# marianaGarcez/SpatialFlink

Hardware: AMD Instinct MI355X
Metric: points/sec per window (kNN k=50, range r) at 1/2/4/8 MI355X; % HBM roofline (higher is better)
Workload: dtype f64

## Files before the change

spatialflink_amd/csrc/k_knn.hip:

```cpp
#define GF_TU_NAME k_knn_hip
#include "gf_buildtag.hpp"

#include <type_traits>

#include "gf_geom.hpp"
#include "gf_internal.hpp"

namespace gf {

__device__ __forceinline__ bool classify_cg(const QueryRect& q, double px, double py) {
  const double xs = (px == px) ? px : q.minX;
  const double ys = (py == py) ? py : q.minY;
  const bool inG = q.g_any && in_iv(q.gx, xs) && in_iv(q.gy, ys);
  return inG || (in_iv(q.cgx, xs) && in_iv(q.cgy, ys));
}

template <int METRIC>
__device__ __forceinline__ bool knn_pass(double qx, double qy, const QueryRect& qr, double px, double py,
                                         double sp, double T) {
  const double dx = qx - px, dy = qy - py;
  const double s = dx * dx + dy * dy;
  if (!(s <= sp)) return false;
  if (!classify_cg(qr, px, py)) return false;
  return METRIC == 0 ? true : fdlibm_hypot(dx, dy) <= T;
}
template <int METRIC>
__device__ __forceinline__ double knn_dist(double qx, double qy, double px, double py) {
  const double dx = qx - px, dy = qy - py;
  return METRIC == 0 ? sqrt(dx * dx + dy * dy) : fdlibm_hypot(dx, dy);
}

__device__ __forceinline__ uint64_t okey(int64_t o) { return (uint64_t)o ^ 0x8000000000000000ull; }
__device__ __forceinline__ int64_t from_okey(uint64_t k) { return (int64_t)(k ^ 0x8000000000000000ull); }

struct RecView {
  gf_knn_header* h;
  double* d;
  int64_t* o;
  int64_t* i;
};
__host__ __device__ inline RecView rec_view(void* base, int k) {
  RecView v;
  v.h = (gf_knn_header*)base;
  v.d = (double*)(v.h + 1);
  v.o = (int64_t*)(v.d + k);
  v.i = v.o + k;
  return v;
}

__device__ void sample_finish(KnnState* st, uint32_t* lh, int32_t k, double r, int metric, int64_t bbase) {
  __shared__ uint32_t wsum[kBlock / 64];
  __shared__ int s_last, s_bin;
  __syncthreads();
  for (int j = threadIdx.x; j < kDistBins; j += kBlock)
    if (lh[j]) atomicAdd(&st->hist[j], lh[j]);
  asm volatile("s_waitcnt vmcnt(0)" ::: "memory");
  __syncthreads();
  if (threadIdx.x == 0) {
    const uint32_t t = atomicAdd(&st->ticket, 1u);
    s_last = (t == gridDim.x - 1);
  }
  __syncthreads();
  if (!s_last) return;
  constexpr int kPer = kDistBins / kBlock;
  uint32_t v[kPer];
  uint32_t s = 0;
#pragma unroll
  for (int j = 0; j < kPer; ++j) {
    v[j] = __hip_atomic_load(&st->hist[threadIdx.x * kPer + j], __ATOMIC_RELAXED, __HIP_MEMORY_SCOPE_AGENT);
    s += v[j];
  }
  const int lane = threadIdx.x & 63, wid = threadIdx.x >> 6;
  uint32_t inc = s;
#pragma unroll
  for (int off = 1; off < 64; off <<= 1) {
    const uint32_t t = __shfl_up(inc, off, 64);
    if (lane >= off) inc += t;
  }
  if (lane == 63) wsum[wid] = inc;
  if (threadIdx.x == 0) s_bin = -1;
  __syncthreads();
  uint32_t before = 0;
  for (int w = 0; w < wid; ++w) before += wsum[w];
  const uint32_t excl = before + inc - s;
  const uint32_t kk = (uint32_t)k;
  if (excl < kk && kk <= excl + s) {
    uint32_t run = excl;
    for (int j = 0; j < kPer; ++j) {
      run += v[j];
      if (run >= kk) { s_bin = threadIdx.x * kPer + j; break; }
    }
  }
  __syncthreads();
  if (threadIdx.x == 0) {
    double T = r;
    if (s_bin >= 0) {
      const double up = dist_bin_upper(s_bin, bbase);
      T = up < r ? up : r;
    }
    st->T = T;
    st->s_pre = s_prefilter(T, metric);
    __hip_atomic_store(&st->ticket, 0u, __ATOMIC_RELAXED, __HIP_MEMORY_SCOPE_AGENT);
  }
  for (int j = threadIdx.x; j < kDistBins; j += kBlock) st->hist[j] = 0u;
}

template <int METRIC>
__global__ __launch_bounds__(kBlock) void knn_sample_kernel(KnnSampleArgs a) {
  __shared__ uint32_t lh[kDistBins];
#ifdef GF_TRACE
  if (blockIdx.x == 0 && threadIdx.x == 0) a.st->tr[0] = wall_clock64();
#endif
  if (a.use_hint) {
    const double h = a.st->hint_T;
    if (h > 0.0) {
      if (blockIdx.x == 0 && threadIdx.x == 0) {
        const double T = h < a.r ? h : a.r;
        a.st->T = T;
        a.st->s_pre = s_prefilter(T, a.metric);
      }
      return;
    }
  }
  constexpr int kPairs = kSamplePerBlock / 2 / kBlock;
  for (int j = threadIdx.x; j < kDistBins; j += kBlock) lh[j] = 0u;
  const int64_t npairs = a.n >> 1;
  const int64_t stride = npairs / gridDim.x;
  const int64_t p0 = (int64_t)blockIdx.x * stride;
  const int64_t bbase = dist_bin_base(a.r);
  double2 xv[kPairs], yv[kPairs];
#pragma unroll
  for (int u = 0; u < kPairs; ++u) {
    const int64_t i = 2 * (p0 + u * kBlock + threadIdx.x);
    xv[u] = *reinterpret_cast<const double2*>(a.x + i);
    yv[u] = *reinterpret_cast<const double2*>(a.y + i);
  }
  __syncthreads();
#pragma unroll
  for (int u = 0; u < kPairs; ++u) {
    if (knn_pass<METRIC>(a.qx, a.qy, a.qr, xv[u].x, yv[u].x, a.s_r, a.r))
      atomicAdd(&lh[dist_bin(knn_dist<METRIC>(a.qx, a.qy, xv[u].x, yv[u].x), bbase)], 1u);
    if (knn_pass<METRIC>(a.qx, a.qy, a.qr, xv[u].y, yv[u].y, a.s_r, a.r))
      atomicAdd(&lh[dist_bin(knn_dist<METRIC>(a.qx, a.qy, xv[u].y, yv[u].y), bbase)], 1u);
  }
  sample_finish(a.st, lh, a.k, a.r, a.metric, bbase);
}

hipError_t launch_knn_sample(gf_ctx* ctx, const KnnSampleArgs& a) {
  KTimer t(ctx, GF_K_KNN_SAMPLE);
  if (a.metric == 0)
    hipLaunchKernelGGL(knn_sample_kernel<0>, dim3(kSampleBlocks), dim3(kBlock), 0, ctx->stream, a);
  else
    hipLaunchKernelGGL(knn_sample_kernel<1>, dim3(kSampleBlocks), dim3(kBlock), 0, ctx->stream, a);
  return hipGetLastError();
}

typedef double dbl2 __attribute__((ext_vector_type(2)));

template <int NT>
__device__ __forceinline__ dbl2 ld2(const dbl2* p) {
  if (NT) return __builtin_nontemporal_load(p);
  return *p;
}

template <class C, class Store>
__device__ __forceinline__ void wave_reserve(C* ctr, bool c, Store&& store) {
  const uint64_t m = __ballot(c);
  if (m == 0) return;
  const int lane = threadIdx.x & 63;
  const int leader = __ffsll((unsigned long long)m) - 1;
  C base = 0;
  if (lane == leader) base = atomicAdd(ctr, (C)__popcll(m));
  base = __shfl(base, leader, 64);
  if (c) store(base + (C)__popcll(m & ((1ull << lane) - 1ull)));
}

__device__ __forceinline__ void wave_append(bool c, double d, uint32_t idx, const KnnScanArgs& a) {
  wave_reserve(&a.st->count, c, [&](unsigned long long pos) {
    if (pos < a.cap) {
      a.cand_d[pos] = d;
      a.cand_i[pos] = idx;
      a.cand_o[pos] = a.objID[idx];
    }
  });
}

template <int METRIC, int U>
__device__ __forceinline__ void knn_scan_tile(const KnnScanArgs& a, const dbl2 (&xv)[U], const dbl2 (&yv)[U],
                                              int64_t p0, int64_t wstride, double sp, double T) {
  uint32_t cm = 0;
#pragma unroll
  for (int u = 0; u < U; ++u) {
    cm |= (uint32_t)knn_pass<METRIC>(a.qx, a.qy, a.qr, xv[u].x, yv[u].x, sp, T) << (2 * u);
    cm |= (uint32_t)knn_pass<METRIC>(a.qx, a.qy, a.qr, xv[u].y, yv[u].y, sp, T) << (2 * u + 1);
  }
  if (__ballot(cm != 0)) {
#pragma unroll
    for (int u = 0; u < U; ++u) {
      const uint32_t i0 = (uint32_t)(2 * (p0 + u * wstride));
      const bool c0 = (cm >> (2 * u)) & 1u, c1 = (cm >> (2 * u + 1)) & 1u;
      wave_append(c0, c0 ? knn_dist<METRIC>(a.qx, a.qy, xv[u].x, yv[u].x) : 0.0, i0, a);
      wave_append(c1, c1 ? knn_dist<METRIC>(a.qx, a.qy, xv[u].y, yv[u].y) : 0.0, i0 + 1, a);
    }
  }
}

__device__ __forceinline__ bool x_in_band(double qx, const dbl2& xv, double sp) {
  const double dx0 = qx - xv.x, dx1 = qx - xv.y;
  return (dx0 * dx0 <= sp) | (dx1 * dx1 <= sp);
}

template <int METRIC, int U, int NT>
__device__ __forceinline__ void knn_scan_tile_x(const KnnScanArgs& a, const dbl2 (&xv)[U], const dbl2* py,
                                                int64_t p0, int64_t wstride, double sp, double T) {
  bool bx[U], any = false;
#pragma unroll
  for (int u = 0; u < U; ++u) {
    bx[u] = x_in_band(a.qx, xv[u], sp);
    any |= bx[u];
  }
  if (__ballot(any) == 0) return;
  dbl2 yv[U];
#pragma unroll
  for (int u = 0; u < U; ++u) {
    yv[u].x = NAN; yv[u].y = NAN;
    if (bx[u]) yv[u] = ld2<NT>(py + u * wstride);
  }
  knn_scan_tile<METRIC, U>(a, xv, yv, p0, wstride, sp, T);
}

template <int METRIC, int U, int NT>
__device__ __forceinline__ void knn_scan_body(const KnnScanArgs& a, double sp, double T, int64_t bid, int64_t nblk) {
  const int lane = threadIdx.x & 63;
  const int64_t wstride = nblk * kBlock;
  const int64_t pbeg = a.begin >> 1;
  const int64_t npf = (a.end - a.begin) >> 1;
  const int64_t iters = npf / (U * wstride);
  const int64_t off = bid * kBlock + (threadIdx.x & ~63) + lane;
  const dbl2* px = reinterpret_cast<const dbl2*>(a.x) + pbeg + off;
  const dbl2* py = reinterpret_cast<const dbl2*>(a.y) + pbeg + off;
#ifdef GF_TRACE
  if (threadIdx.x == 0) atomicMin(&a.st->tr[1], (unsigned long long)wall_clock64());
#endif
  dbl2 xv[U];
  if (iters > 0) {
#pragma unroll
    for (int u = 0; u < U; ++u) xv[u] = ld2<NT>(px + u * wstride);
  }
  for (int64_t it = 0; it < iters; ++it) {
    dbl2 xn[U];
    px += U * wstride;
    if (it + 1 < iters) {
#pragma unroll
      for (int u = 0; u < U; ++u) xn[u] = ld2<NT>(px + u * wstride);
    } else {
#pragma unroll
      for (int u = 0; u < U; ++u) { xn[u].x = NAN; xn[u].y = NAN; }
    }
    knn_scan_tile_x<METRIC, U, NT>(a, xv, py, pbeg + off + it * U * wstride, wstride, sp, T);
    py += U * wstride;
#pragma unroll
    for (int u = 0; u < U; ++u) xv[u] = xn[u];
  }
  const int64_t pend = (a.end + 1) >> 1;
  for (int64_t p = pbeg + iters * U * wstride + off; p - lane < pend; p += wstride) {
    const int64_t i = 2 * p;
    dbl2 xt[1], yt[1];
    const bool pair = i + 1 < a.end;
    if (pair) {
      xt[0] = *reinterpret_cast<const dbl2*>(a.x + i);
    } else {
      xt[0].x = i < a.end ? a.x[i] : NAN;
      xt[0].y = NAN;
    }
    yt[0].x = NAN; yt[0].y = NAN;
    const bool bx = x_in_band(a.qx, xt[0], sp);
    if (__ballot(bx) == 0) continue;
    if (bx) {
      if (pair) yt[0] = *reinterpret_cast<const dbl2*>(a.y + i);
      else yt[0].x = a.y[i];
    }
    knn_scan_tile<METRIC, 1>(a, xt, yt, p, wstride, sp, T);
  }
#ifdef GF_TRACE
  __syncthreads();
  if (threadIdx.x == 0) atomicMax(&a.st->tr[2], (unsigned long long)wall_clock64());
#endif
}

template <int METRIC, int U, int NT>
__global__ __launch_bounds__(kBlock) void knn_scan_kernel(KnnScanArgs a) {
  const double sp = a.use_state ? a.st->s_pre : a.s_pre;
  const double T = a.use_state ? a.st->T : a.T;
  knn_scan_body<METRIC, U, NT>(a, sp, T, blockIdx.x, gridDim.x);
}

template <int METRIC>
static void launch_scan_u(gf_ctx* ctx, const KnnScanArgs& a, int blocks, int unroll, int nt) {
  const dim3 g(blocks), b(kBlock);
#define GF_SCAN(U, N) hipLaunchKernelGGL((knn_scan_kernel<METRIC, U, N>), g, b, 0, ctx->stream, a)
  if (nt) {
    if (unroll <= 1) GF_SCAN(1, 1); else if (unroll == 2) GF_SCAN(2, 1); else if (unroll <= 4) GF_SCAN(4, 1); else GF_SCAN(8, 1);
  } else {
    if (unroll <= 1) GF_SCAN(1, 0); else if (unroll == 2) GF_SCAN(2, 0); else if (unroll <= 4) GF_SCAN(4, 0); else GF_SCAN(8, 0);
  }
#undef GF_SCAN
}

hipError_t launch_knn_scan(gf_ctx* ctx, const KnnScanArgs& a, int blocks, int unroll, int nt) {
  KTimer t(ctx, GF_K_KNN_SCAN);
  if (a.metric == 0) launch_scan_u<0>(ctx, a, blocks, unroll, nt);
  else launch_scan_u<1>(ctx, a, blocks, unroll, nt);
  return hipGetLastError();
}

constexpr int kSelT = 256;
static_assert(kSelT == kBlock, "the fused kernel's select block is a scan-sized block");

struct SelFull {
  static constexpr int kCap = 1024, kHBits = 11, kK = kMaxK;
  uint64_t sd[kCap], so[kCap];
  int64_t si[kCap];
  uint64_t rd[kK], ro[kK];
  int64_t ri[kK];
  union {
    uint32_t hist[kDistBins];
    struct {
      uint64_t rund[kSelT], runo[kSelT];
      int64_t runi[kSelT];
      uint64_t hkey[1 << kHBits];
      uint32_t hpos[1 << kHBits];
    };
  };
  uint32_t wsum[kSelT / 64];
  int s_cnt, s_bin, s_maxpos;
  uint32_t s_S, s_below;
  unsigned long long s_rng[4];
};
struct SelLite {
  static constexpr int kCap = 256, kHBits = 9, kK = 256;
  uint64_t sd[kCap], so[kCap];
  int64_t si[kCap];
  uint64_t rd[kK], ro[kK];
  int64_t ri[kK];
  union {
    uint32_t hist[kDistBins];
    struct {
      uint64_t rund[kSelT], runo[kSelT];
      int64_t runi[kSelT];
      uint64_t hkey[1 << kHBits];
      uint32_t hpos[1 << kHBits];
    };
  };
  uint32_t wsum[kSelT / 64];
  int s_cnt, s_bin, s_maxpos;
  uint32_t s_S, s_below;
  unsigned long long s_rng[4];
};
static_assert(SelFull::kCap > kMaxK, "the general path needs room for the running list plus a chunk");
static_assert(sizeof(SelLite) <= 29 * 1024, "fused kernel: 5 blocks per CU must fit the LDS");

__device__ __forceinline__ bool kless(uint64_t ad, uint64_t ao, int64_t ai, uint64_t bd, uint64_t bo, int64_t bi) {
  if (ad != bd) return ad < bd;
  if (ao != bo) return ao < bo;
  return ai < bi;
}

__device__ __forceinline__ void wave_bitonic(uint64_t& d, uint64_t& o, int64_t& i) {
  const int lane = threadIdx.x & 63;
#pragma unroll
  for (int size = 2; size <= 64; size <<= 1) {
#pragma unroll
    for (int stride = size >> 1; stride > 0; stride >>= 1) {
      const uint64_t pd = __shfl_xor(d, stride, 64), po = __shfl_xor(o, stride, 64);
      const int64_t pi = __shfl_xor(i, stride, 64);
      const bool up = (lane & size) == 0;
      const bool lower = (lane & stride) == 0;
      const bool plt = kless(pd, po, pi, d, o, i);
      if ((lower == up) ? plt : !plt) { d = pd; o = po; i = pi; }
    }
  }
}

template <class LDS>
__device__ void sort_regs(LDS& L, uint64_t d, uint64_t o, int64_t i) {
  const int tid = threadIdx.x, lane = tid & 63, w = tid >> 6;
  wave_bitonic(d, o, i);
  L.rund[tid] = d; L.runo[tid] = o; L.runi[tid] = i;
  __syncthreads();
  if (i != INT64_MAX) {
    int rank = lane;
#pragma unroll
    for (int v = 0; v < kSelT / 64; ++v) {
      if (v == w) continue;
      int lo = 0;
#pragma unroll
      for (int step = 32; step > 0; step >>= 1) {
        const int m = 64 * v + lo + step - 1;
        if (kless(L.rund[m], L.runo[m], L.runi[m], d, o, i)) lo += step;
      }
      if (lo == 63 && kless(L.rund[64 * v + 63], L.runo[64 * v + 63], L.runi[64 * v + 63], d, o, i)) lo = 64;
      rank += lo;
    }
    L.sd[rank] = d; L.so[rank] = o; L.si[rank] = i;
  }
  __syncthreads();
}

template <class LDS>
__device__ void bitonic_lds(LDS& L, int P) {
  for (int size = 2; size <= P; size <<= 1) {
    for (int stride = size >> 1; stride > 0; stride >>= 1) {
      for (int t = threadIdx.x; t < (P >> 1); t += kSelT) {
        const int i = 2 * stride * (t / stride) + (t & (stride - 1));
        const int j = i + stride;
        const bool up = (i & size) == 0;
        if (kless(L.sd[j], L.so[j], L.si[j], L.sd[i], L.so[i], L.si[i]) == up) {
          uint64_t td = L.sd[i]; L.sd[i] = L.sd[j]; L.sd[j] = td;
          uint64_t to = L.so[i]; L.so[i] = L.so[j]; L.so[j] = to;
          int64_t ti = L.si[i]; L.si[i] = L.si[j]; L.si[j] = ti;
        }
      }
      __syncthreads();
    }
  }
}

__device__ __forceinline__ int pow2ceil(int v) {
  int p = 2;
  while (p < v) p <<= 1;
  return p;
}

template <class LDS>
__device__ void sort_lds(LDS& L, int cnt) {
  if (cnt <= kSelT) {
    const int tid = threadIdx.x;
    const bool in = tid < cnt;
    const uint64_t d = in ? L.sd[tid] : ~0ull, o = in ? L.so[tid] : ~0ull;
    const int64_t i = in ? L.si[tid] : INT64_MAX;
    __syncthreads();
    sort_regs(L, d, o, i);
  } else {
    const int P = pow2ceil(cnt);
    for (int t = cnt + threadIdx.x; t < P; t += kSelT) { L.sd[t] = ~0ull; L.so[t] = ~0ull; L.si[t] = INT64_MAX; }
    __syncthreads();
    bitonic_lds(L, P);
  }
}

template <class LDS>
__device__ int dedupe_topk(LDS& L, int cnt, int k) {
  constexpr int kH = 1 << LDS::kHBits;
  constexpr int kR = LDS::kCap / kSelT;
  const int tid = threadIdx.x, lane = tid & 63, w = tid >> 6;
  for (int s = tid; s < kH; s += kSelT) { L.hkey[s] = ~0ull; L.hpos[s] = 0xFFFFFFFFu; }
  if (tid == 0) L.s_maxpos = 0x7FFFFFFF;
  __syncthreads();
  uint32_t slot[kR];
#pragma unroll
  for (int r = 0; r < kR; ++r) {
    const int p = r * kSelT + tid;
    slot[r] = 0;
    if (p < cnt) {
      const uint64_t o = L.so[p];
      if (o == ~0ull) {
        atomicMin(&L.s_maxpos, p);
        slot[r] = kH;
      } else {
        uint32_t h = (uint32_t)((o * 0x9E3779B97F4A7C15ull) >> (64 - LDS::kHBits));
        for (;;) {
          const unsigned long long prev = atomicCAS((unsigned long long*)&L.hkey[h], ~0ull, o);
          if (prev == ~0ull || prev == o) break;
          h = (h + 1) & (kH - 1);
        }
        atomicMin(&L.hpos[h], (uint32_t)p);
        slot[r] = h;
      }
    }
  }
  __syncthreads();
  int base = 0;
#pragma unroll
  for (int r = 0; r < kR; ++r) {
    if (r * kSelT < cnt && base < k) {
      const int p = r * kSelT + tid;
      bool keep = false;
      if (p < cnt) keep = (slot[r] == (uint32_t)kH) ? (L.s_maxpos == p) : (L.hpos[slot[r]] == (uint32_t)p);
      const uint64_t m = __ballot(keep);
      if (lane == 0) L.wsum[w] = (uint32_t)__popcll(m);
      __syncthreads();
      int before = base;
      for (int v = 0; v < w; ++v) before += (int)L.wsum[v];
      const int total = (int)(L.wsum[0] + L.wsum[1] + L.wsum[2] + L.wsum[3]);
      const int pos = before + __popcll(m & ((1ull << lane) - 1ull));
      if (keep && pos < k) { L.rd[pos] = L.sd[p]; L.ro[pos] = L.so[p]; L.ri[pos] = L.si[p]; }
      base += total;
      __syncthreads();
    }
  }
  return base < k ? base : k;
}

template <class LDS>
__device__ __forceinline__ void lds_push(LDS& L, bool c, uint64_t d, uint64_t o, int64_t i) {
  wave_reserve(&L.s_cnt, c, [&](int pos) { L.sd[pos] = d; L.so[pos] = o; L.si[pos] = i; });
}

template <class LDS>
__device__ void kth_bin(LDS& L, uint32_t target, uint32_t base) {
  const int tid = threadIdx.x, lane = tid & 63, wid = tid >> 6;
  constexpr int kB = kDistBins / kSelT;
  uint32_t v[kB], s = 0;
#pragma unroll
  for (int j = 0; j < kB; ++j) { v[j] = L.hist[kB * tid + j]; s += v[j]; }
  uint32_t inc = s;
#pragma unroll
  for (int off = 1; off < 64; off <<= 1) {
    const uint32_t t = __shfl_up(inc, off, 64);
    if (lane >= off) inc += t;
  }
  if (lane == 63) L.wsum[wid] = inc;
  __syncthreads();
  const uint32_t total = L.wsum[0] + L.wsum[1] + L.wsum[2] + L.wsum[3];
  uint32_t before = 0;
  for (int w = 0; w < wid; ++w) before += L.wsum[w];
  const uint32_t excl = before + inc - s;
  if (target > total) {
    if (tid == kSelT - 1) { L.s_bin = kDistBins - 1; L.s_S = base + total; L.s_below = base + total - v[kB - 1]; }
  } else if (excl < target && target <= excl + s) {
    uint32_t run = excl;
    for (int j = 0; j < kB; ++j) {
      run += v[j];
      if (run >= target) { L.s_bin = kB * tid + j; L.s_S = base + run; L.s_below = base + run - v[j]; break; }
    }
  }
  __syncthreads();
}

#ifdef GF_TRACE
#define GF_TR(j) do { if (threadIdx.x == 0) tr[j] = wall_clock64(); } while (0)
#else
#define GF_TR(j) do { } while (0)
#endif

template <class LDS, bool GENERAL>
__device__ void knn_select_body(const KnnSelectArgs& a, LDS& L) {
  const int tid = threadIdx.x;
  const int lane = tid & 63;
  const int k = a.k;
  constexpr int kPer = LDS::kCap / kSelT;
#ifdef GF_TRACE
  uint64_t* tr = (uint64_t*)((char*)a.result + sizeof(gf_knn_header) + 24 * (size_t)k);
#endif
  GF_TR(0);
  const unsigned long long count = a.st->count;
  const double T = a.use_state ? a.st->T : a.T;
  double dv[kPer];
  uint32_t iv[kPer];
  int64_t ov[kPer];
#pragma unroll
  for (int j = 0; j < kPer; ++j) {
    const int64_t i = tid + (int64_t)j * kSelT;
    const bool in = (unsigned long long)i < a.cap;
    dv[j] = in ? a.cand_d[i] : 0.0;
    iv[j] = in ? a.cand_i[i] : 0u;
    ov[j] = in ? a.cand_o[i] : 0;
  }
  const bool overflow = count > a.cap;
  const int64_t M = overflow ? 0 : (int64_t)count;
  bool done = overflow;
  int nres = 0;
  GF_TR(1);

  if (!overflow && M <= kSelT) {
    const bool in = tid < M;
    sort_regs(L, in ? dbits(dv[0]) : ~0ull, in ? okey(ov[0]) : ~0ull, in ? (int64_t)iv[0] : INT64_MAX);
    GF_TR(4);
    nres = dedupe_topk(L, (int)M, k);
    done = true;
    GF_TR(5);
  } else if (!overflow) {
    for (int i = tid; i < kDistBins; i += kSelT) L.hist[i] = 0u;
    if (tid == 0) { L.s_cnt = 0; }
    __syncthreads();
    const int64_t bbase = dist_bin_base(T);
    constexpr int kU = GENERAL ? 4 : 2;
    auto each_of = [&](auto&& f, auto with_oi) {
#pragma unroll
      for (int j = 0; j < kPer; ++j) f(tid + (int64_t)j * kSelT < M, dv[j], ov[j], iv[j]);
      for (int64_t i0 = LDS::kCap; i0 < M; i0 += (int64_t)kU * kSelT) {
        double d[kU];
        int64_t o[kU];
        uint32_t x[kU];
#pragma unroll
        for (int u = 0; u < kU; ++u) {
          const int64_t i = i0 + (int64_t)u * kSelT + tid;
          const bool in = i < M;
          d[u] = in ? a.cand_d[i] : 0.0;
          o[u] = in && decltype(with_oi)::value ? a.cand_o[i] : 0;
          x[u] = in && decltype(with_oi)::value ? a.cand_i[i] : 0u;
        }
#pragma unroll
        for (int u = 0; u < kU; ++u) f(i0 + (int64_t)u * kSelT + tid < M, d[u], o[u], x[u]);
      }
    };
    auto each = [&](auto&& f) { each_of(f, std::true_type{}); };
    each_of([&](bool v, double d, int64_t, uint32_t) {
      if (v) atomicAdd(&L.hist[dist_bin(d, bbase)], 1u);
    }, std::false_type{});
    __syncthreads();
    GF_TR(2);
    kth_bin(L, (uint32_t)k, 0u);
    GF_TR(3);
    const int bstar = L.s_bin;
    uint64_t cut_d = ~0ull, cut_o = ~0ull;
    if (L.s_S > (uint32_t)LDS::kCap) {
      uint64_t r0 = ~0ull, r1 = 0ull, r2 = ~0ull, r3 = 0ull;
      each([&](bool v, double d, int64_t o, uint32_t) {
        if (v && dist_bin(d, bbase) == bstar) {
          const uint64_t db = dbits(d), ok = okey(o);
          r0 = db < r0 ? db : r0; r1 = db > r1 ? db : r1;
          r2 = ok < r2 ? ok : r2; r3 = ok > r3 ? ok : r3;
        }
      });
#pragma unroll
      for (int off = 1; off < 64; off <<= 1) {
        const uint64_t t0 = __shfl_xor(r0, off, 64), t1 = __shfl_xor(r1, off, 64);
        const uint64_t t2 = __shfl_xor(r2, off, 64), t3 = __shfl_xor(r3, off, 64);
        r0 = t0 < r0 ? t0 : r0; r1 = t1 > r1 ? t1 : r1; r2 = t2 < r2 ? t2 : r2; r3 = t3 > r3 ? t3 : r3;
      }
      if (tid == 0) { L.s_rng[0] = ~0ull; L.s_rng[1] = 0ull; L.s_rng[2] = ~0ull; L.s_rng[3] = 0ull; }
      for (int i = tid; i < kDistBins; i += kSelT) L.hist[i] = 0u;
      __syncthreads();
      if (lane == 0) {
        atomicMin(&L.s_rng[0], r0); atomicMax(&L.s_rng[1], r1);
        atomicMin(&L.s_rng[2], r2); atomicMax(&L.s_rng[3], r3);
      }
      __syncthreads();
      const bool tie = L.s_rng[0] == L.s_rng[1];
      const uint64_t kmin = tie ? L.s_rng[2] : L.s_rng[0], span = (tie ? L.s_rng[3] : L.s_rng[1]) - kmin;
      const int bits = span ? 64 - __clzll((long long)span) : 0;
      const int shift = bits > 12 ? bits - 12 : 0;
      each([&](bool v, double d, int64_t o, uint32_t) {
        if (v && dist_bin(d, bbase) == bstar) atomicAdd(&L.hist[((tie ? okey(o) : dbits(d)) - kmin) >> shift], 1u);
      });
      __syncthreads();
      const uint32_t below = L.s_below;
      kth_bin(L, (uint32_t)k - below, below);
      const int b2 = L.s_bin;
      const uint64_t cut = b2 >= kDistBins - 1 ? ~0ull : kmin + ((((uint64_t)b2 + 1ull) << shift) - 1ull);
      cut_d = tie ? L.s_rng[0] : cut;
      cut_o = tie ? cut : ~0ull;
    }
    if (L.s_S <= (uint32_t)LDS::kCap) {
      each([&](bool v, double d, int64_t o, uint32_t x) {
        const int b = dist_bin(d, bbase);
        const uint64_t ok = okey(o);
        const bool c = v && (b < bstar || (b == bstar && dbits(d) <= cut_d && ok <= cut_o));
        lds_push(L, c, dbits(d), ok, (int64_t)x);
      });
      __syncthreads();
      GF_TR(4);
      const int cnt = L.s_cnt;
#ifdef GF_TRACE
      if (tid == 0) tr[8] = (uint64_t)cnt;
#endif
      sort_lds(L, cnt);
      nres = dedupe_topk(L, cnt, k);
      done = (nres >= k) || (cnt == M);
      GF_TR(5);
    }
    if (GENERAL && !done) {
      int nr = 0;
      uint64_t md = ~0ull, mo = ~0ull;
      int64_t mi = INT64_MAX;
      for (int64_t i0 = 0; i0 < M; i0 += kSelT) {
        for (int i = tid; i < nr; i += kSelT) { L.sd[i] = L.rd[i]; L.so[i] = L.ro[i]; L.si[i] = L.ri[i]; }
        if (tid == 0) L.s_cnt = nr;
        __syncthreads();
        const int64_t i = i0 + tid;
        bool c = i < M;
        uint64_t d = 0, o = 0;
        int64_t ix = 0;
        if (c) {
          d = dbits(a.cand_d[i]);
          o = okey(a.cand_o[i]);
          ix = (int64_t)a.cand_i[i];
          c = nr < k || kless(d, o, ix, md, mo, mi);
        }
        lds_push(L, c, d, o, ix);
        __syncthreads();
        const int cnt = L.s_cnt;
        if (cnt > nr) {
          sort_lds(L, cnt);
          nr = dedupe_topk(L, cnt, k);
          if (nr == k) { md = L.rd[k - 1]; mo = L.ro[k - 1]; mi = L.ri[k - 1]; }
        }
        __syncthreads();
      }
      nres = nr;
      done = true;
    }
  }
  const bool too_few = done && !overflow && nres < k && T < a.r;
  const int status = (!done || overflow || too_few) ? 1 : 0;
  GF_TR(6);
#ifdef GF_TRACE
  if (tid == 0) {
    tr[9] = a.st->tr[0]; tr[10] = a.st->tr[1]; tr[11] = a.st->tr[2];
    a.st->tr[1] = ~0ull; a.st->tr[2] = 0ull;
  }
#endif
  RecView out = rec_view(a.result, k);
  if (status == 0)
    for (int i = tid; i < nres; i += kSelT) {
      out.d[i] = from_bits(L.rd[i]); out.o[i] = from_okey(L.ro[i]); out.i[i] = L.ri[i] + a.idx_base;
    }
  if (tid == 0) {
    out.h->status = status;
    out.h->n = status ? 0 : nres;
    out.h->k = k;
    out.h->flags = overflow ? 1 : 0;
    out.h->candidates = (int64_t)count;
    out.h->threshold = T;
    a.st->count = 0ull;
    a.st->maybe = 0ull;
    if (a.write_hint) {
      double h;
      if (status == 0) h = nres == k ? fmax(2.0 * from_bits(L.rd[k - 1]), 4.9e-324) : a.r;
      else if (overflow) h = T * sqrt(0.5 * (double)a.cap / (double)count);
      else if (too_few) h = 2.0 * T;
      else h = T;
      a.st->hint_T = h;
    }
  }
}

__global__ __launch_bounds__(kSelT) void knn_select_kernel(KnnSelectArgs a) {
  __shared__ SelFull L;
  knn_select_body<SelFull, true>(a, L);
}

__device__ __forceinline__ int64_t large_count(const KnnLargeArgs& a, int which) {
  const int64_t c = (int64_t)a.cnt[which];
  return c < a.m ? c : a.m;
}

__global__ __launch_bounds__(kBlock) void knn_large_key_kernel(KnnLargeArgs a) {
  const int64_t m = large_count(a, a.pass);
  for (int64_t j = (int64_t)blockIdx.x * kBlock + threadIdx.x; j < m; j += (int64_t)gridDim.x * kBlock) {
    const uint32_t p = a.perm[j];
    uint32_t v;
    switch (a.field) {
      case 0: v = a.ci[p]; break;
      case 1: v = lo32(a.cd[p]); break;
      case 2: v = hi32(a.cd[p]); break;
      case 3: v = (uint32_t)(uint64_t)a.co[p]; break;
      default: v = (uint32_t)((uint64_t)a.co[p] >> 32) ^ 0x80000000u; break;
    }
    a.keys[j] = v;
  }
}

__global__ __launch_bounds__(kBlock) void knn_large_iota_kernel(KnnLargeArgs a) {
  const int64_t m = large_count(a, 0);
  for (int64_t j = (int64_t)blockIdx.x * kBlock + threadIdx.x; j < m; j += (int64_t)gridDim.x * kBlock)
    a.perm[j] = (uint32_t)j;
}

__global__ void knn_large_start_kernel(KnnLargeArgs a) {
  a.cnt[0] = (uint32_t)*a.lane_count;
  a.cnt[1] = 0u;
  *a.lane_count = 0ull;
  *a.lane_maybe = 0ull;
}

__global__ __launch_bounds__(kBlock) void knn_large_first_kernel(KnnLargeArgs a) {
  const int64_t m = large_count(a, 0);
  const int lane = threadIdx.x & 63;
  const int64_t stride = (int64_t)gridDim.x * kBlock;
  for (int64_t j0 = (int64_t)blockIdx.x * kBlock + (threadIdx.x & ~63); j0 < m; j0 += stride) {
    const int64_t j = j0 + lane;
    uint32_t p = 0u;
    bool first = false;
    if (j < m) {
      p = a.perm[j];
      first = j == 0 || a.co[p] != a.co[a.perm[j - 1]];
    }
    wave_reserve(&a.cnt[1], first, [&](uint32_t pos) { a.out[pos] = p; });
  }
}

__global__ __launch_bounds__(kBlock) void knn_large_record_kernel(KnnLargeArgs a) {
  gf_knn_header* h = reinterpret_cast<gf_knn_header*>(a.result);
  const int32_t k = a.k;
  const int32_t n = (int64_t)a.cnt[1] < (int64_t)k ? (int32_t)a.cnt[1] : k;
  double* rd = reinterpret_cast<double*>(h + 1);
  int64_t* ro = reinterpret_cast<int64_t*>(rd + k);
  int64_t* ri = ro + k;
  for (int64_t j = (int64_t)blockIdx.x * kBlock + threadIdx.x; j < n; j += (int64_t)gridDim.x * kBlock) {
    const uint32_t p = a.perm[j];
    rd[j] = a.cd[p];
    ro[j] = a.co[p];
    ri[j] = (int64_t)a.ci[p] + a.idx_base;
  }
  if (blockIdx.x == 0 && threadIdx.x == 0) {
    h->status = 0;
    h->n = n;
    h->k = k;
    h->flags = 0;
    h->candidates = a.cnt[0];
    h->threshold = a.T;
  }
}

static unsigned large_blocks(int64_t items) {
  const int64_t b = (items + kBlock - 1) / kBlock;
  return (unsigned)(b < 1 ? 1 : (b > 2048 ? 2048 : b));
}

hipError_t launch_knn_large(gf_ctx* ctx, int op, const KnnLargeArgs& a) {
  hipStream_t s = ctx->stream;
  const dim3 g(large_blocks(a.m)), b(kBlock);
  switch (op) {
    case 0: hipLaunchKernelGGL(knn_large_iota_kernel, g, b, 0, s, a); break;
    case 1: hipLaunchKernelGGL(knn_large_key_kernel, g, b, 0, s, a); break;
    case 2: hipLaunchKernelGGL(knn_large_first_kernel, g, b, 0, s, a); break;
    case 5: hipLaunchKernelGGL(knn_large_start_kernel, dim3(1), dim3(1), 0, s, a); break;
    default: hipLaunchKernelGGL(knn_large_record_kernel, dim3(large_blocks(a.k)), b, 0, s, a); break;
  }
  return hipGetLastError();
}

hipError_t launch_knn_select(gf_ctx* ctx, const KnnSelectArgs& a) {
  KTimer t(ctx, GF_K_KNN_SELECT);
  hipLaunchKernelGGL(knn_select_kernel, dim3(1), dim3(kSelT), 0, ctx->stream, a);
  return hipGetLastError();
}

struct StridedRecs {
  const char* base;
  size_t stride;
  __device__ const char* operator()(int r) const { return base + (size_t)r * stride; }
};
struct ListRecs {
  const KnnRecList* l;
  __device__ const char* operator()(int r) const { return l->rec[r]; }
};

template <class LDS, class Src>
__device__ void knn_merge_body(int32_t k, const Src& src, int32_t nrec, void* result, LDS& L, int foreign = 0) {
  __shared__ int s_off[kMaxMergeRecs + 1], s_status, s_foreign;
  const int tid = threadIdx.x;
  if (tid == 0) {
    s_foreign = 0;
    int off = 0, st = 0;
    for (int r = 0; r < nrec; ++r) {
      const gf_knn_header* h = (const gf_knn_header*)src(r);
      s_off[r] = off;
      off += h->status == 0 ? h->n : 0;
      st = h->status > st ? h->status : st;
    }
    s_off[nrec] = off;
    s_status = st;
  }
  __syncthreads();
  int nr = 0, r = 0;
  while (r < nrec) {
    for (int i = tid; i < nr; i += kSelT) { L.sd[i] = L.rd[i]; L.so[i] = L.ro[i]; L.si[i] = L.ri[i]; }
    int cnt = nr;
    while (r < nrec && cnt + (s_off[r + 1] - s_off[r]) <= LDS::kCap) {
      RecView in = rec_view((void*)src(r), k);
      const int n = s_off[r + 1] - s_off[r];
      for (int i = tid; i < n; i += kSelT) {
        const int64_t o = in.o[i];
        L.sd[cnt + i] = dbits(in.d[i]); L.so[cnt + i] = okey(o); L.si[cnt + i] = in.i[i];
        if (foreign && o < GF_OBJID_NUMERIC_MIN && o != GF_OBJID_NULL) s_foreign = 1;
      }
      cnt += n;
      ++r;
    }
// ... 649 lines not shown
```

Measured before the change: 796.2 billion.

## Fuse small-candidate sort with hash dedupe and use DPP lane swaps in bitonic

The wave bitonic sort now exchanges lanes with DPP and permlane swaps in place of __shfl_xor, and kless becomes a branchless comparison. For the full layout, the cross-wave merge rank runs its binary searches over the three other waves in lockstep to expose more independent LDS loads. In the general path with at most 256 candidates, a fused sort_dedupe_regs uses an LDS hash table with atomicCAS/atomicMin to keep the first rank per object and bitmask popcounts to compact the top-k, replacing the separate dedupe_topk pass. This aims to cut selection latency and barriers, at the cost of atomic contention, hash probing, and reliance on gfx950 permlane builtins.

Result: no change. 790.7 billion (-0.7%).

```diff
diff --git a/spatialflink_amd/csrc/k_knn.hip b/spatialflink_amd/csrc/k_knn.hip
--- a/spatialflink_amd/csrc/k_knn.hip
+++ b/spatialflink_amd/csrc/k_knn.hip
@@ -319,6 +319,7 @@
 
 struct SelFull {
   static constexpr int kCap = 1024, kHBits = 11, kK = kMaxK;
+  static constexpr bool kLockstep = true;
   uint64_t sd[kCap], so[kCap];
   int64_t si[kCap];
   uint64_t rd[kK], ro[kK];
@@ -339,6 +340,7 @@
 };
 struct SelLite {
   static constexpr int kCap = 256, kHBits = 9, kK = 256;
+  static constexpr bool kLockstep = false;
   uint64_t sd[kCap], so[kCap];
   int64_t si[kCap];
   uint64_t rd[kK], ro[kK];
@@ -361,35 +363,84 @@
 static_assert(sizeof(SelLite) <= 29 * 1024, "fused kernel: 5 blocks per CU must fit the LDS");
 
 __device__ __forceinline__ bool kless(uint64_t ad, uint64_t ao, int64_t ai, uint64_t bd, uint64_t bo, int64_t bi) {
-  if (ad != bd) return ad < bd;
-  if (ao != bo) return ao < bo;
-  return ai < bi;
+  const bool dl = ad < bd, de = ad == bd, ol = ao < bo, oe = ao == bo, il = ai < bi;
+  return dl | (de & (ol | (oe & il)));
+}
+
+template <int CTRL>
+__device__ __forceinline__ uint32_t dpp_mov(uint32_t v) {
+  return (uint32_t)__builtin_amdgcn_mov_dpp((int)v, CTRL, 0xf, 0xf, true);
+}
+template <int STRIDE>
+__device__ __forceinline__ uint32_t lane_xor32(uint32_t v, int lane) {
+  constexpr int kQuadXor1 = 0xB1, kQuadXor2 = 0x4E, kQuadRev = 0x1B, kRowMirror = 0x140, kHalfMirror = 0x141;
+  if constexpr (STRIDE == 1) return dpp_mov<kQuadXor1>(v);
+  else if constexpr (STRIDE == 2) return dpp_mov<kQuadXor2>(v);
+  else if constexpr (STRIDE == 4) return dpp_mov<kQuadRev>(dpp_mov<kHalfMirror>(v));
+  else if constexpr (STRIDE == 8) return dpp_mov<kHalfMirror>(dpp_mov<kRowMirror>(v));
+  else if constexpr (STRIDE == 16) {
+    const auto r = __builtin_amdgcn_permlane16_swap(v, v, false, false);
+    return (lane & 16) ? r[0] : r[1];
+  } else {
+    static_assert(STRIDE == 32, "a wave has 64 lanes");
+    const auto r = __builtin_amdgcn_permlane32_swap(v, v, false, false);
+    return (lane & 32) ? r[0] : r[1];
+  }
+}
+template <int STRIDE>
+__device__ __forceinline__ uint64_t lane_xor(uint64_t v, int lane) {
+  return (uint64_t)lane_xor32<STRIDE>((uint32_t)(v >> 32), lane) << 32 | lane_xor32<STRIDE>((uint32_t)v, lane);
+}
+
+template <int SIZE, int STRIDE>
+__device__ __forceinline__ void bitonic_steps(uint64_t& d, uint64_t& o, int64_t& i, int lane) {
+  const uint64_t pd = lane_xor<STRIDE>(d, lane), po = lane_xor<STRIDE>(o, lane);
+  const int64_t pi = (int64_t)lane_xor<STRIDE>((uint64_t)i, lane);
+  const bool up = (lane & SIZE) == 0;
+  const bool lower = (lane & STRIDE) == 0;
+  const bool plt = kless(pd, po, pi, d, o, i);
+  if ((lower == up) ? plt : !plt) { d = pd; o = po; i = pi; }
+  if constexpr (STRIDE > 1) bitonic_steps<SIZE, STRIDE / 2>(d, o, i, lane);
 }
 
 __device__ __forceinline__ void wave_bitonic(uint64_t& d, uint64_t& o, int64_t& i) {
   const int lane = threadIdx.x & 63;
-#pragma unroll
-  for (int size = 2; size <= 64; size <<= 1) {
-#pragma unroll
-    for (int stride = size >> 1; stride > 0; stride >>= 1) {
-      const uint64_t pd = __shfl_xor(d, stride, 64), po = __shfl_xor(o, stride, 64);
-      const int64_t pi = __shfl_xor(i, stride, 64);
-      const bool up = (lane & size) == 0;
-      const bool lower = (lane & stride) == 0;
-      const bool plt = kless(pd, po, pi, d, o, i);
-      if ((lower == up) ? plt : !plt) { d = pd; o = po; i = pi; }
-    }
-  }
+  bitonic_steps<2, 1>(d, o, i, lane);
+  bitonic_steps<4, 2>(d, o, i, lane);
+  bitonic_steps<8, 4>(d, o, i, lane);
+  bitonic_steps<16, 8>(d, o, i, lane);
+  bitonic_steps<32, 16>(d, o, i, lane);
+  bitonic_steps<64, 32>(d, o, i, lane);
 }
 
 template <class LDS>
-__device__ void sort_regs(LDS& L, uint64_t d, uint64_t o, int64_t i) {
-  const int tid = threadIdx.x, lane = tid & 63, w = tid >> 6;
-  wave_bitonic(d, o, i);
-  L.rund[tid] = d; L.runo[tid] = o; L.runi[tid] = i;
-  __syncthreads();
-  if (i != INT64_MAX) {
-    int rank = lane;
+__device__ __forceinline__ int merged_rank(const LDS& L, uint64_t d, uint64_t o, int64_t i, int lane, int w) {
+  int rank = lane;
+  if constexpr (LDS::kLockstep) {
+    constexpr int kF = kSelT / 64 - 1;
+    int base[kF], lo[kF];
+    bool all[kF];
+#pragma unroll
+    for (int u = 0; u < kF; ++u) {
+      base[u] = 64 * ((w + 1 + u) & (kSelT / 64 - 1));
+      lo[u] = 0;
+      const int m = base[u] + 63;
+      all[u] = kless(L.rund[m], L.runo[m], L.runi[m], d, o, i);
+    }
+#pragma unroll
+    for (int step = 32; step > 0; step >>= 1) {
+      bool below[kF];
+#pragma unroll
+      for (int u = 0; u < kF; ++u) {
+        const int m = base[u] + lo[u] + step - 1;
+        below[u] = kless(L.rund[m], L.runo[m], L.runi[m], d, o, i);
+      }
+#pragma unroll
+      for (int u = 0; u < kF; ++u) lo[u] += below[u] ? step : 0;
+    }
+#pragma unroll
+    for (int u = 0; u < kF; ++u) rank += all[u] ? 64 : lo[u];
+  } else {
 #pragma unroll
     for (int v = 0; v < kSelT / 64; ++v) {
       if (v == w) continue;
@@ -402,9 +453,68 @@
       if (lo == 63 && kless(L.rund[64 * v + 63], L.runo[64 * v + 63], L.runi[64 * v + 63], d, o, i)) lo = 64;
       rank += lo;
     }
+  }
+  return rank;
+}
+
+template <class LDS>
+__device__ void sort_regs(LDS& L, uint64_t d, uint64_t o, int64_t i) {
+  const int tid = threadIdx.x, lane = tid & 63, w = tid >> 6;
+  wave_bitonic(d, o, i);
+  L.rund[tid] = d; L.runo[tid] = o; L.runi[tid] = i;
+  __syncthreads();
+  if (i != INT64_MAX) {
+    const int rank = merged_rank(L, d, o, i, lane, w);
     L.sd[rank] = d; L.so[rank] = o; L.si[rank] = i;
   }
   __syncthreads();
+}
+
+template <class LDS>
+__device__ int sort_dedupe_regs(LDS& L, uint64_t d, uint64_t o, int64_t i, int k) {
+  constexpr int kHB = 9, kH = 1 << kHB;
+  static_assert(kHB <= LDS::kHBits && kH >= 2 * kSelT, "load factor <= 1/2 inside the layout's table");
+  const int tid = threadIdx.x, lane = tid & 63, w = tid >> 6;
+  for (int s = tid; s < kH; s += kSelT) { L.hkey[s] = ~0ull; L.hpos[s] = 0xFFFFFFFFu; }
+  if (tid < 4) L.s_rng[tid] = 0ull;
+  if (tid == 0) L.s_maxpos = 0x7FFFFFFF;
+  wave_bitonic(d, o, i);
+  L.rund[tid] = d; L.runo[tid] = o; L.runi[tid] = i;
+  __syncthreads();
+  int rank = -1;
+  uint32_t slot = 0;
+  if (i != INT64_MAX) {
+    rank = merged_rank(L, d, o, i, lane, w);
+    if (o == ~0ull) {
+      atomicMin(&L.s_maxpos, rank);
+      slot = kH;
+    } else {
+      uint32_t h = (uint32_t)((o * 0x9E3779B97F4A7C15ull) >> (64 - kHB));
+      for (;;) {
+        const unsigned long long prev = atomicCAS((unsigned long long*)&L.hkey[h], ~0ull, o);
+        if (prev == ~0ull || prev == o) break;
+        h = (h + 1) & (kH - 1);
+      }
+      atomicMin(&L.hpos[h], (uint32_t)rank);
+      slot = h;
+    }
+  }
+  __syncthreads();
+  bool keep = false;
+  if (rank >= 0) keep = (slot == (uint32_t)kH) ? (L.s_maxpos == rank) : (L.hpos[slot] == (uint32_t)rank);
+  if (keep) atomicOr(&L.s_rng[rank >> 6], 1ull << (rank & 63));
+  __syncthreads();
+  int total = 0, pos = 0;
+#pragma unroll
+  for (int v = 0; v < kSelT / 64; ++v) {
+    const unsigned long long m = L.s_rng[v];
+    total += __popcll(m);
+    if (v < (rank >> 6)) pos += __popcll(m);
+    else if (v == (rank >> 6)) pos += __popcll(m & ((1ull << (rank & 63)) - 1ull));
+  }
+  if (keep && pos < k) { L.rd[pos] = d; L.ro[pos] = o; L.ri[pos] = i; }
+  __syncthreads();
+  return total < k ? total : k;
 }
 
 template <class LDS>
@@ -575,9 +685,16 @@
 
   if (!overflow && M <= kSelT) {
     const bool in = tid < M;
-    sort_regs(L, in ? dbits(dv[0]) : ~0ull, in ? okey(ov[0]) : ~0ull, in ? (int64_t)iv[0] : INT64_MAX);
-    GF_TR(4);
-    nres = dedupe_topk(L, (int)M, k);
+    const uint64_t kd = in ? dbits(dv[0]) : ~0ull, ko = in ? okey(ov[0]) : ~0ull;
+    const int64_t ki = in ? (int64_t)iv[0] : INT64_MAX;
+    if constexpr (GENERAL) {
+      GF_TR(4);
+      nres = sort_dedupe_regs(L, kd, ko, ki, k);
+    } else {
+      sort_regs(L, kd, ko, ki);
+      GF_TR(4);
+      nres = dedupe_topk(L, (int)M, k);
+    }
     done = true;
     GF_TR(5);
   } else if (!overflow) {
```
